# f90/Wave-U-Net

Measured on AMD Instinct MI355X. Metric: waveform samples/sec fwd+bwd, M1 12-level Wave-U-Net @1/2/4/8 GPU, higher is better.
Workload: dtype f32

## Files before the change

wave-u-net_amd/csrc/wun_dispatch.hip:

```cpp
#include "wun_plan_impl.h"

#include <algorithm>
#include <cstdio>
#include <cstdlib>
#include <cstring>
#include <functional>
#include <string>
#include <vector>

ConvArgs conv_base(const wun_plan* p) {
    ConvArgs a;
    memset(&a, 0, sizeof(a));
    a.B = p->B; a.ostride = 1; a.loader = LOADER_DIRECT;
    return a;
}
void set_src0(ConvArgs& a, const float* ws, const Buf& b, int off, int C) {
    a.src0 = ws + b.off; a.bs0 = b.bs; a.pitch0 = b.pitch; a.off0 = off; a.C0 = C;
}
void set_src1(ConvArgs& a, const float* ws, const Buf& b, int off, int C) {
    a.src1 = ws + b.off; a.bs1 = b.bs; a.pitch1 = b.pitch; a.off1 = off; a.C1 = C;
}
void set_dst0(ConvArgs& a, float* ws, const Buf& b, int off, const Buf* mask) {
    a.dst0 = ws + b.off; a.obs0 = b.bs; a.opitch0 = b.pitch; a.ooff0 = off;
    a.msk0 = mask ? ws + mask->off : nullptr;
// ... 155 lines not shown
                }
                vec[idx] = bc;
                if (p->sw.tune_log)
                    fprintf(stderr, "[tune conv-bf16 %s#%zu] C=%d N=%d T=%d K=%d ld=%d ph2=%d cands=%d base %.3f ms -> code=%d %.3f ms\n",
                            p->in_bwd ? "bwd" : "fwd", idx, a.C0 + a.C1, a.N, a.Tout, a.KW, a.loader, (a.flags & F_PHASE2) ? 1 : 0, n,
                            base, bc.variant, best);
            }
            if (p->tune_mode >= 1 && idx < vec.size() && vec[idx].variant >= kBf16VariantBase && conv_bf16_choice_ok(a, vec[idx].variant))
                a.force_variant = vec[idx].variant + 1;
            return launch_conv_bf16(a, s, p->sw);
        }
    }
    if (p->tune_mode == 1) {
        if (vec.size() <= idx) vec.resize(idx + 1, ConvChoice{-1, 0});
        std::vector<ConvChoice> cands_v(640);
        std::vector<float> tms_v(641);
        ConvChoice* cands = cands_v.data();
        float* tms = tms_v.data();
        const int n = conv_list_candidates(a, part ? cap : 0, cands, 640, p->sw);
        time_candidates(p, s, n + 1, [&](int i) {
            ConvArgs b = a;
            b.ups_y = nullptr; b.ubw_dz = nullptr;
            if (i < n) { b.force_variant = cands[i].variant + 1; b.force_ksplit = cands[i].ksplit; }
            return launch_conv(b, part, cap, s, p->sw);
        }, tms);
        const float base = tms[n];
        float best = base;
        ConvChoice bc{-1, 0};
        int bi = -1;
        for (int i = 0; i < n; ++i)
            if (bi < 0 ? tms[i] < 1e29f : tms[i] < tms[bi]) bi = i;
        if (bi >= 0 && tms[bi] < base * 0.98f) { best = tms[bi]; bc = cands[bi]; }
        vec[idx] = bc;
        char head[96];
        snprintf(head, sizeof(head), "%s %zu %d %d %.4f\n", p->in_bwd ? "cb" : "cf", idx, -1, 0, base);
        tune_alts(p, head, tms, (size_t)n, best, base, [&](FILE* f, size_t i) {
            fprintf(f, "%s %zu %d %d %.4f\n", p->in_bwd ? "cb" : "cf", idx, cands[i].variant, cands[i].ksplit, tms[i]);
        });
        if (p->sw.tune_log)
            fprintf(stderr, "[tune conv %s#%zu] C=%d N=%d T=%d K=%d ld=%d ph2=%d cands=%d base %.3f ms -> v=%d ks=%d %.3f ms\n",
                    p->in_bwd ? "bwd" : "fwd", idx, a.C0 + a.C1, a.N, a.Tout, a.KW, a.loader, (a.flags & F_PHASE2) ? 1 : 0, n,
                    base, bc.variant, bc.ksplit, best);
    }
    if (p->tune_mode >= 1 && idx < vec.size() && vec[idx].variant >= 0 &&
        conv_choice_ok(a, part ? cap : 0, vec[idx].variant, vec[idx].ksplit > 0 ? vec[idx].ksplit : 1, p->sw)) {
        a.force_variant = vec[idx].variant + 1; a.force_ksplit = vec[idx].ksplit;
    }
    return launch_conv(a, part, cap, s, p->sw);
}

static bool wgrad_common_geom(WgradArgs* parts, int nparts, int mtw, int nw) {
    int m0 = 0, n0 = 0;
    for (int i = 0; i < nparts; ++i) {
        parts[i].force_mtw = mtw; parts[i].force_nw = nw;
        int m, n;
        wgrad_resolved_geom(parts[i], m, n);
        if (i == 0) { m0 = m; n0 = n; }
        else if (m != m0 || n != n0) return false;
    }
    return true;
}

int run_wgrad(const wun_plan* p, WgradArgs* parts, int nparts, const ConvLayer& cl, float* ws,
                     float* grads, hipStream_t main, hipStream_t s, bool dep, bool accum) {
    if (dep) {
        int rcd = stream_dep(p, main, s);
        if (rcd) return rcd;
    }
    if (p->bf16) {
        if (!wgrad_bf16_supported(parts[0])) return fail(WUN_ERR_UNSUPPORTED, "bf16 mode: weight-gradient shape not served by the bf16 kernel");
        for (int i = 0; i < nparts; ++i) { parts[i].bf16 = 1; parts[i].sbf = 1; }
// ... 186 lines not shown
```

wave-u-net_amd/csrc/wun_internal.h:

```cpp
#pragma once
#include <hip/hip_runtime.h>
#include <stdint.h>
#include <string>

namespace wun {

enum { LOADER_DIRECT = 0, LOADER_DEINT = 1 };

enum WunEarlyWindow { EW_DEFAULT, EW_OFF, EW_DEEP, EW_ALL };
enum WunEventScope { EV_DEFAULT, EV_SYSTEM, EV_DEVICE };
enum WunSidePrio { PRIO_DEFAULT, PRIO_LOW, PRIO_HIGH, PRIO_NORMAL };
struct WunSwitches {
    bool no_dedup = false;
    WunEarlyWindow early_window = EW_DEFAULT;
    bool odd_fuse_set = false;
    int odd_fuse_min = 64;
    bool no_odd_align = false;
    bool no_fuse_ups = false;
    bool bf16_head_serial = false;
    bool single_stream = false;
    WunSidePrio side_prio = PRIO_DEFAULT;
    WunEventScope event_scope = EV_DEFAULT;
    bool no_win = false;
    bool no_narrow = false;
    bool no_narrow_down0 = false;
    bool no_narrow_stream = false;
    int narrow_splits = 0;
    bool no_dma = false;
    bool no_k3 = false;
    int win_tk = 64;
    int bf16_lds_cap = 80;
    int tune_rounds = 4;
    bool tune_log = false;
    std::string tune_alts;
    int tune_alts_max = 6;
    float tune_alts_tol = 1.15f;
    bool dump_layout = false;
    bool profile_detail = false;
    bool win_occ = false;
};
WunSwitches wun_switches_from_env();

enum { F_LRELU = 1, F_ACCUM = 2, F_VEC4 = 4, F_PHASE2 = 8 };

struct ConvArgs {
    const float* src0; const float* src1;
    long long bs0, bs1;
    int pitch0, pitch1;
    int off0, off1;
    int C0, C1;
    int Tin;
    int shift;
// ... 7 lines not shown
    int opitch0, opitch1;
    int ooff0, ooff1;
    const float* msk0; const float* msk1;
    int ostride;
    int Tout;
    float* dec; long long decbs; int decpitch;
    int dec_exp; int dec_lo; unsigned dec_len;
    float* dec1; long long dec1bs; int dec1pitch;
    int dec_off, dec1_off;
    int flags;
    int B;
    int loader;
    int Tlim;
    int kw_full;
    int force_variant;
    int force_ksplit;
    int cps;
    float* part;
    int wb_c8p, wb_npad;
    int acc_lo; unsigned acc_len;
    float* ups_y; long long ups_bs; int ups_pitch; int ups_tup; const float* ups_w;
    float* ubw_dz; const float* ubw_x; long long ubw_bs; int ubw_pitch; int ubw_n;
    int xbf, obf;
};
#define WUN_FIRST_RETIRED_VARIANT 42
#define WUN_NUM_RETIRED_VARIANTS 14
int conv_last_fused_ups();
static inline bool aligned16(const void* p) { return (reinterpret_cast<uintptr_t>(p) & 15) == 0; }
void conv_output_setup(ConvArgs& a);

struct WgradArgs {
    const float* src0; const float* src1;
    long long bs0, bs1;
    int pitch0, pitch1;
    int off0, off1;
    int C0, C1;
    int Tin;
    int shift;
    int KW;
    int loader;
    const float* dz; long long dzbs; int dzpitch; int N; int Tq;
    float* out;
    int direct;
    int split_base;
    int nsplit; int units_per_split; int nQT; int B;
    int ablate;
    int force_mtw, force_nw;
// ... 81 lines not shown
    int C, B, Tin;
    const float* dpre; long long dps, dpbs; int dppitch;
    const float* Wh; long long hoff[4]; int Sh, Ko, padl, Tfeat, Tout, moff_feat;
    const float* dlast; int moff_diff;
    float* dmix;
};

struct PackDesc {
    long long src_off;
    long long dst_off;
    int KW, C, N, C8p, Npad;
    int src_in_ws;
};

struct WtDesc {
    long long src_off;
    long long dst_off;
    int J, C, N, k_last, k_step;
    int mode;
};

size_t conv_lds_bytes(const ConvArgs& a, int variant, const WunSwitches& sw);
int  conv_pick_variant(const ConvArgs& a);
hipError_t launch_conv(const ConvArgs& a, float* part, long long part_cap, hipStream_t s, const WunSwitches& sw);
double conv_flops(const ConvArgs& a);
long long conv_natural_wgs_phase2(const ConvArgs& a);
int conv_list_candidates(const ConvArgs& a, long long part_cap, ConvChoice* out, int maxn, const WunSwitches& sw);
bool conv_choice_ok(const ConvArgs& a, long long part_cap, int variant, int ksplit, const WunSwitches& sw);
int conv_num_variants();
int wgrad_max_units(const WgradArgs& a, const WunSwitches& sw);

int  wgrad_pick_nsplit(const WgradArgs& a, const WunSwitches& sw);
hipError_t launch_wgrad(const WgradArgs& a, hipStream_t s, const WunSwitches& sw);
void wgrad_resolved_geom(const WgradArgs& a, int& mtw, int& nw);
long long wgrad_partial_floats(const WgradArgs& a, const WunSwitches& sw);
hipError_t launch_wgrad_reduce(const WgradArgs& a, const float* partial, int nsplit, float* out_w, float* out_b,
                               hipStream_t s, const WunSwitches& sw);
enum { EW_UPSAMPLE = 0, EW_UPSAMPLE_BWD, EW_INTERP_GRAD, EW_HEAD_FWD, EW_HEAD_DFEAT, EW_BTC_TO_NCW, EW_NUM_OPS };
enum { EW_PATH_NONE = 0, EW_PATH_SCALAR, EW_PATH_VEC4, EW_PATH_VEC8_BF16, EW_PATH_ONE_STAGE, EW_PATH_TWO_STAGE,
       EW_PATH_GENERIC, EW_PATH_FOUR_POSITION };
int elementwise_last_path(int op);
hipError_t launch_upsample(const UpsampleArgs& a, hipStream_t s);
hipError_t launch_upsample_bwd(const UpsampleBwdArgs& a, hipStream_t s);
hipError_t launch_interp_grad(const UpsampleBwdArgs& a, hipStream_t s, bool accum = false);
hipError_t launch_head_fwd_off(const HeadArgs& a, const long long* hoff, hipStream_t s);
int head_bwd_blocks(const HeadArgs& a);
hipError_t launch_head_bwd_off(const HeadArgs& a, const long long* hoff, hipStream_t s);
// ... 78 lines not shown
```

wave-u-net_amd/csrc/wun_kernels.hip:

```cpp
#include "wun_device.h"

#include <cstdio>
#include <cstdlib>
#include <map>
#include <mutex>
#include <string>
#include <algorithm>
#include <vector>

namespace wun {

__device__ __forceinline__ f32x4 mfma16(float a, float b, f32x4 c) {
    return __builtin_amdgcn_mfma_f32_16x16x4f32(a, b, c, 0, 0, 0);
}

__host__ __device__ static inline int fit_pitch(int width, int mod32) {
    return width + (((mod32 - (width % 32)) % 32) + 32) % 32;
}

struct ProfSlot { std::string name; std::string tag; double flops; double bytes; hipEvent_t e0, e1, c0, c1; };
static std::vector<ProfSlot> g_prof;
static bool g_prof_on = false;
static bool g_prof_detail = false;
static std::mutex g_prof_mu;
// ... 72 lines not shown
    }
    g_prof.clear();
    double overhead_ms = 0.0;
    if (!empty_ms.empty()) {
        std::sort(empty_ms.begin(), empty_ms.end());
        overhead_ms = empty_ms[empty_ms.size() / 2];
    }
    char obuf[96];
    snprintf(obuf, sizeof(obuf), "{\"bracket_overhead_ms\": %.6f, ", overhead_ms);
    std::string out = std::string(obuf) + "\"launches\": [" + detail + "], \"kernels\": [";
    bool first = true;
    for (auto& kv : agg) {
        char buf[512];
        snprintf(buf, sizeof(buf), "%s{\"name\": \"%s\", \"launches\": %ld, \"ms\": %.6f, \"flops\": %.6e, \"bytes\": %.6e}",
                 first ? "" : ", ", kv.first.c_str(), kv.second.n, kv.second.ms, kv.second.flops, kv.second.bytes);
        out += buf;
        first = false;
    }
    out += "]}";
    return out;
}

#define WUN_JMAX 15


__device__ __forceinline__ int fast_div(int n, int d, float inv) {
    int q = (int)(((float)n + 0.5f) * inv);
    const int r = n - q * d;
    q += (r >= d) ? 1 : 0;
    q -= (r < 0) ? 1 : 0;
    return q;
}

#define WUN_FOLD_XCAP(TT) (3 * (TT) + 32)

__device__ __forceinline__ void conv_copy1(const ConvArgs& a, int b, int n, int q, float v) {
    if (a.dec != nullptr) {
        float* row = a.dec + (long long)b * a.decbs + (long long)n * a.decpitch + a.dec_off;
        if (a.dec_exp) {
            const unsigned pos = (unsigned)(2 * q - a.dec_lo);
            if (pos < a.dec_len) row[pos] = v;
        } else if ((q & 1) == 0) {
            row[q >> 1] = v;
        }
    }
    if (a.dec1 != nullptr && (q & 1) != 0) a.dec1[(long long)b * a.dec1bs + (long long)n * a.dec1pitch + a.dec1_off + (q >> 1)] = v;
// ... 23 lines not shown
    extern __shared__ __attribute__((aligned(16))) float lds_all[];
    const int kg = KG > 1 ? __builtin_amdgcn_readfirstlane((int)(threadIdx.x >> 8)) : 0;
    constexpr int TT = WT * MT * 16;
    constexpr int NT = WN * NW * 16;
    constexpr int NT4 = NT / 4;
    constexpr int CH = CK / 2;
    constexpr int TPR = 256 / CK;
    constexpr int XIT_D = FOLD ? (WUN_FOLD_XCAP(TT) + TPR - 1) / TPR : (TT + WUN_JMAX - 1 + TPR - 1) / TPR;
    constexpr int TPC = 256 / CH;
    constexpr int XIT_I = FOLD ? (2 * WUN_FOLD_XCAP(TT) + TPC - 1) / TPC
                               : (2 * (TT + (WUN_JMAX + 1) / 2 - 1) + TPC - 1) / TPC;
    constexpr int XIT = XVEC ? 1 : (XIT_D > XIT_I ? XIT_D : XIT_I);
    constexpr int WIT = XVEC ? 1 : (WUN_JMAX * CK * NT4 + 255) / 256;
    constexpr int XDIT = XVEC ? (CK * ((TT + 48) / 4) + 255) / 256 : 1;
    constexpr int WDIT = XVEC ? (WUN_JMAX * CK * (NT4 + 4) + 255) / 256 : 1;
    static_assert(!(XVEC && FOLD), "DMA staging is not implemented for batch-folded tiles");

    const int XB = CK * XP, LB = CK * XP + J * CK * WP;
    float* lds = lds_all + (KG > 1 ? kg * 2 * LB : 0);
    float* Xs = lds;
    float* Ws = lds + XB;

    const int tid = KG > 1 ? (int)(threadIdx.x & 255) : (int)threadIdx.x;
    const int lane = tid & 63;
    const int li = lane & 15, lg = lane >> 4;
    const int wave = __builtin_amdgcn_readfirstlane(tid >> 6);
#define WUN_PRIO_HI() __builtin_amdgcn_s_setprio(2)
#define WUN_PRIO_LO() __builtin_amdgcn_s_setprio(0)
    WUN_PRIO_HI();
    int bid = xcd_contiguous_block((int)blockIdx.x, (int)gridDim.x);
    const int nt = bid % nNT; bid /= nNT;
    const int tt = bid % nTT; bid /= nTT;
    const float inv_tout = 1.0f / (float)a.Tout;
    const int b = FOLD ? fast_div(tt * TT, a.Tout, inv_tout) : bid % a.B;
    const int ksg = FOLD ? bid : bid / a.B;
    const int ksp = ksg * KG + kg;
    const int q0 = tt * TT, n0 = nt * NT;
    int fold_nb = 1;
    const int fold_seg = a.Tout + J - 1;
    if constexpr (FOLD) {
        int last = fast_div(q0 + TT - 1, a.Tout, inv_tout);
        if (last > a.B - 1) last = a.B - 1;
        fold_nb = last - b + 1;
    }
    const int wt0 = (wave % WT) * MT * 16;
    const int wn0 = (wave / WT) * NW * 16;
// ... 19 lines not shown

    float xreg[XIT];
    f32x4 wreg[WIT];
    unsigned xmask = 0, wmask = 0;

    int xt[XIT];
    unsigned xmask_s = 0, wmask_s = 0;
    const int xrow = deint ? tid / TPC : tid / TPR;
    const int dl0 = XVEC ? (((a.off0 - a.shift) % 4) + 4) % 4 : 0;
    const int dl1 = (XVEC && a.C1 > 0) ? (((a.off1 - a.shift) % 4) + 4) % 4 : dl0;
    int xdo[XDIT], wdo[WDIT];
    int nvr = 1, e00 = 0, e01 = 0;
    bool xedge = false;
    const float* vb0 = a.src0 + (long long)b * a.bs0;
    const float* vb1 = (a.src1 != nullptr) ? a.src1 + (long long)b * a.bs1 : vb0;
    const int XG = XP >> 2, WG4 = WP >> 2;
    if constexpr (XVEC) {
        const int tbase = q0 - a.shift;
        nvr = (UW + (dl0 > dl1 ? dl0 : dl1) + 3) >> 2;
        e00 = a.off0 + tbase - dl0;
        e01 = a.off1 + tbase - dl1;
        const int tf0 = tbase - dl0, tf1 = tbase - dl1;
        xedge = tf0 < 0 || tf0 + 4 * nvr > a.Tin || (a.C1 > 0 && (tf1 < 0 || tf1 + 4 * nvr > a.Tin));
        const float inv_xg = 1.0f / (float)XG;
#pragma unroll
        for (int i = 0; i < XDIT; ++i) {
            const int f = tid + i * 256;
            const int row = fast_div(f, XG, inv_xg), g = f - row * XG;
            xdo[i] = (row < CK && g < nvr) ? (row << 20) | (4 * g) : -1;
        }
        const float inv_wg = 1.0f / (float)WG4;
#pragma unroll
        for (int i = 0; i < WDIT; ++i) {
            const int f = tid + i * 256;
            const int row = fast_div(f, WG4, inv_wg), c4 = f - row * WG4;
            const int j = row / CK, r = row - j * CK;
            const bool ok = j < J && c4 < NT4;
            int wo;
            if (!phase2) {
                int col = n0 + c4 * 4;
                col = col > a.N - 4 ? a.N - 4 : col;
                wo = (j * Ctot + r) * a.N + col;
            } else {
                const int x = c4 * 4, ph = x / (NT / 2), cl = x % (NT / 2);
                int col = n0h + cl;
                col = col > a.N - 4 ? a.N - 4 : col;
                wo = (j * Ctot + r) * (2 * a.N) + ph * a.N + col;
            }
            wdo[i] = ok ? wo : -1;
        }
    }
    if constexpr (!XVEC) {
        const int lr = deint ? tid % TPC : tid % TPR;
        const int stride_i = deint ? TPC : TPR;
        const int lim = deint ? 2 * UW : UW;
        const int tbase = (deint ? 2 * q0 : q0) - a.shift;
        const int seglen = deint ? 2 * fold_seg : fold_seg;
        const float inv_seglen = 1.0f / (float)seglen;
#pragma unroll
        for (int i = 0; i < XIT; ++i) {
            const int u = lr + i * stride_i;
            int t = tbase + u, bl = 0;
            if constexpr (FOLD) { bl = fast_div(u, seglen, inv_seglen); t = u - bl * seglen - a.shift; }
            const bool ok = u < lim && t >= 0 && t < a.Tin;
            int tc = t < 0 ? 0 : t;
            if (tc > a.Tin - 1) tc = a.Tin - 1;
            if constexpr (FOLD) {
                if (bl > fold_nb - 1) bl = fold_nb - 1;
                tc |= bl << 20;
            }
            xt[i] = tc;
            xmask_s |= (ok ? 1u : 0u) << i;
// ... 678 lines not shown
    if (!aligned16(a.src0) || (a.bs0 & 3) != 0 || (a.pitch0 & 3) != 0 || a.pitch0 < 4) return false;
    if (a.src1 != nullptr && (!aligned16(a.src1) || (a.bs1 & 3) != 0 || (a.pitch1 & 3) != 0 || a.pitch1 < 4)) return false;
    if (a.off0 < 0 || a.off1 < 0 || !aligned16(a.W)) return false;
    if ((long long)cv.CK * a.pitch0 >= (1ll << 31) || (long long)cv.CK * a.pitch1 >= (1ll << 31)) return false;
    return true;
}

static void conv_geom(const ConvArgs& a, int variant, const WunSwitches& sw, int& TT, int& NT, int& J, int& XP, int& WP) {
    const ConvVariant& v = kConvVariants[variant];
    TT = v.WT * v.MT * 16;
    NT = v.WN * v.NW * 16;
    J = conv_J(a);
    XP = fit_pitch(v.fold ? WUN_FOLD_XCAP(TT) : TT + J - 1, 16);
    if (conv_xvec_ok(a, variant, sw)) XP = conv_dma_pitch(TT + J - 1 + 3);
    WP = fit_pitch(NT, 16);
}

static inline long long conv_mtiles(const ConvArgs& a, int variant, int TT, int& bfac) {
    if (kConvVariants[variant].fold) { bfac = 1; return ((long long)a.B * a.Tout + TT - 1) / TT; }
    bfac = a.B;
    return (a.Tout + TT - 1) / TT;
}

size_t conv_lds_bytes(const ConvArgs& a, int variant, const WunSwitches& sw) {
    if (is_k3(variant)) {
        const int bv = conv_tile_variant(variant);
        const size_t stage = WUN_KG * conv_lds_bytes(a, bv, sw);
        const size_t red = (size_t)(WUN_KG - 1) * kConvVariants[bv].MT * kConvVariants[bv].NW * 256 * 16;
        return stage > red ? stage : red;
    }
    if (variant >= WUN_FIRST_RETIRED_VARIANT) return (size_t)1 << 30;
    int TT, NT, J, XP, WP;
    conv_geom(a, variant, sw, TT, NT, J, XP, WP);
    const int CK = kConvVariants[variant].CK;
    return 2 * sizeof(float) * ((size_t)CK * XP + (size_t)J * CK * WP);
}

double conv_flops(const ConvArgs& a) {
    if (a.flags & F_PHASE2)
        return 2.0 * a.kw_full * (double)(a.C0 + a.C1) * a.N * (double)a.Tin * a.B;
    return 2.0 * a.KW * (double)(a.C0 + a.C1) * a.N * (double)a.Tout * a.B;
}

void conv_splitk(const ConvArgs& a, int variant, const WunSwitches& sw, long long part_cap_floats, int& ksplit, int& cps) {
    int TT, NT, J, XP, WP;
    conv_geom(a, variant, sw, TT, NT, J, XP, WP);
// ... 43 lines not shown
        const int CKC = a.loader == LOADER_DEINT ? CK / 2 : CK;
        const int nchunks = (a.C0 + a.C1 + CKC - 1) / CKC;
        int want = a.force_ksplit > nchunks ? nchunks : a.force_ksplit;
        if (part == nullptr) want = 1;
        const long long per = (long long)a.B * a.N * ((a.Tout + 3) & ~3);
        if (want > 1 && (long long)want * per > part_cap) return hipErrorInvalidValue;
        cps = (nchunks + want - 1) / want;
        ksplit = (nchunks + cps - 1) / cps;
    }
    if (KG > 1) {
        const int CKC = a.loader == LOADER_DEINT ? CK / 2 : CK;
        const int nchunks = (a.C0 + a.C1) / CKC;
        const int want = (a.force_ksplit > 0 && part != nullptr) ? a.force_ksplit : 1;
        if ((a.C0 + a.C1) % CKC != 0 || nchunks % (KG * want) != 0) return hipErrorInvalidValue;
        const long long per = (long long)a.B * a.N * ((a.Tout + 3) & ~3);
        if (want > 1 && (long long)want * per > part_cap) return hipErrorInvalidValue;
        ksplit = want;
        cps = nchunks / (KG * want);
    }
    a.cps = cps;
    a.part = ksplit > 1 ? part : nullptr;
    const long long grid = (long long)nTT * nNT * bfac * ksplit;
    if (grid <= 0) return hipSuccess;
    char nm[64];
    snprintf(nm, sizeof(nm), "conv_mfma_kernel<%d, %d, %d, %d, %d, %s%s%s%s>", MT, NW, WT, WN, CK, VECW ? "true" : "false",
             FOLD ? ", fold" : "", XVEC ? ", dma" : "", KG > 1 ? ", k3" : "");
    {
        char tag[160];
        snprintf(tag, sizeof(tag), "C=%d N=%d T=%d K=%d ld=%d B=%d ks=%d ph2=%d acc=%d os=%d grid=%lld", a.C0 + a.C1, a.N,
                 a.Tout, a.KW, a.loader, a.B, ksplit, (a.flags & F_PHASE2) ? 1 : 0, (a.flags & F_ACCUM) ? 1 : 0,
                 a.ostride, grid);
        ProfScope ps(nm, conv_flops(a), s, tag);
        hipLaunchKernelGGL(kern, dim3((unsigned)grid), dim3(256 * KG), lds_launch, s, a, nTT, nNT, J, XP, WP);
    }
    hipError_t e = hipGetLastError();
    if (e != hipSuccess || ksplit == 1) return e;
    const long long total = (long long)a.B * a.N * (((a.Tout + 3) & ~3) >> 2);
    long long blocks = (total + 255) / 256;
    if (blocks > 4096) blocks = 4096;
    {
        const double elems = (double)a.B * a.N * a.Tout;
        double by = 4.0 * elems * (ksplit + 1 + (a.msk0 != nullptr ? 1 : 0) + ((a.flags & F_ACCUM) ? 1 : 0));
        if (a.ups_y != nullptr) by += 4.0 * (double)a.B * a.N * a.ups_tup;
        ProfScope ps("conv_splitk_epilogue_kernel", 0.0, s, "", by);
        hipLaunchKernelGGL(conv_splitk_epilogue_kernel, dim3((unsigned)blocks), dim3(256), 0, s, a, ksplit);
    }
// ... 48 lines not shown

int conv_list_candidates(const ConvArgs& a, long long part_cap, ConvChoice* out, int maxn, const WunSwitches& sw) {
    int n = 0;
    const int nvar = conv_num_variants();
    static const int ks_menu[] = {1, 2, 3, 4, 6, 8, 12, 16, 24, 32, 48};
    for (int v = 0; v < nvar && n < maxn; ++v)
        for (unsigned i = 0; i < sizeof(ks_menu) / sizeof(ks_menu[0]) && n < maxn; ++i) {
            if (!conv_choice_ok(a, part_cap, v, ks_menu[i], sw)) {
                if (is_k3(v) && ks_menu[i] < 8) continue;
                break;
            }
            out[n].variant = v; out[n].ksplit = ks_menu[i]; ++n;
        }
    return n;
}

static_assert(sizeof(kConvVariants) / sizeof(kConvVariants[0]) == WUN_FIRST_RETIRED_VARIANT, "the retired index range follows the tile table");
static int first_k3_variant() { return WUN_FIRST_RETIRED_VARIANT + WUN_NUM_RETIRED_VARIANTS; }
int conv_num_variants() { return first_k3_variant() + kNumK3; }


int conv_last_fused_ups() { return t_last_fused_ups; }

hipError_t launch_conv(const ConvArgs& a_in, float* part, long long part_cap, hipStream_t s, const WunSwitches& sw) {
    ConvArgs a = a_in;
    t_last_fused_ups = 0;
    if (a.ups_y != nullptr && (a.dst1 != nullptr || a.msk0 != nullptr || a.ostride != 1 || a.ooff0 != 0 ||
                               (a.flags & (F_ACCUM | F_PHASE2)) != 0 || a.N0 != a.N || !aligned16(a.ups_y)))
        return hipErrorInvalidValue;
    if (a.ubw_dz != nullptr && (a.dst1 == nullptr || a.msk1 != nullptr || a.ostride != 1 || a.bias != nullptr ||
                                (a.flags & (F_ACCUM | F_PHASE2 | F_LRELU)) != 0 || a.N0 >= a.N || a.ubw_x == nullptr))
        return hipErrorInvalidValue;
    conv_output_setup(a);
    if (conv_J(a) > WUN_JMAX) return hipErrorInvalidValue;
    if (a.KW <= 0) {
        const long long total = (long long)a.B * a.N * (((a.Tout + 3) & ~3) >> 2);
        if (total <= 0) return hipSuccess;
        long long blocks = (total + 255) / 256;
        if (blocks > 4096) blocks = 4096;
        hipLaunchKernelGGL(conv_splitk_epilogue_kernel, dim3((unsigned)blocks), dim3(256), 0, s, a, 0);
        return hipGetLastError();
    }
    const bool vecw = (a.N & 3) == 0 && aligned16(a.W);
    if ((a.flags & F_PHASE2) && !(a.ostride == 1 && a.dst1 == nullptr && vecw)) return hipErrorInvalidValue;
    int v = (a.flags & F_PHASE2) ? conv_pick_variant_phase2(a) : conv_pick_variant(a);
    if (a.force_variant > 0 && vecw) {
        v = a.force_variant - 1;
        if (!conv_choice_ok(a, part != nullptr ? part_cap : 0, v, a.force_ksplit > 0 ? a.force_ksplit : 1, sw)) return hipErrorInvalidValue;
    }
// ... 567 lines not shown
```

wave-u-net_amd/csrc/wun_op.hip:

```cpp
#include "wun_plan_impl.h"

#include <algorithm>
#include <cstdio>
#include <cstdlib>
#include <cstring>

namespace wun {
hipError_t launch_make_wt_one(const float* src, float* dst, WtDesc d, hipStream_t s);
}

static const long long kOpScratchFloats = 8ll << 20;
static int g_op_variant = -1, g_op_ksplit = 0;
static int g_op_wg_mtw = 0, g_op_wg_nw = 0, g_op_wg_nsplit = 0;
static int g_op_wg_bf16 = 0;
static int g_op_wg_narrow = 0;
static int g_op_wg_win = 0;
static float* g_op_copy0 = nullptr; static float* g_op_copy1 = nullptr;
static int g_op_copy_t0 = 0, g_op_copy_t1 = 0, g_op_copy_exp = 0, g_op_copy_lo = 0, g_op_copy_len = 0, g_op_acc_lo = 0, g_op_acc_len = 0;
static float* g_op_ups_y = nullptr; static const float* g_op_ups_w = nullptr;
static int g_op_ups_pitch = 0, g_op_ups_tup = 0;
static thread_local int t_op_epilogue_path = WUN_PATH_NONE;
static float* op_scratch() {
    static float* buf = nullptr;
    if (!buf && hipMalloc((void**)&buf, kOpScratchFloats * sizeof(float)) != hipSuccess) {
// ... 4 lines not shown
}

static void* op_bf16_tmp(int slot, size_t bytes) {
    static void* buf[2] = {nullptr, nullptr};
    static size_t cap[2] = {0, 0};
    if (bytes > cap[slot]) {
        (void)hipDeviceSynchronize();
        if (buf[slot]) (void)hipFree(buf[slot]);
        buf[slot] = nullptr; cap[slot] = 0;
        const size_t want = bytes + (bytes >> 2) + 4096;
        if (hipMalloc(&buf[slot], want) != hipSuccess) { (void)hipGetLastError(); return nullptr; }
        cap[slot] = want;
    }
    return buf[slot];
}
static inline int pad8(int t) { return (t + 7) / 8 * 8; }
static const float* op_to_bf16(int slot, const float* src, long long rows, int T, long long spitch, hipStream_t s) {
    void* dst = op_bf16_tmp(slot, (size_t)rows * pad8(T) * 2 + 64);
    if (!dst) return nullptr;
    if (launch_cast_rows_bf16(src, dst, rows, T, spitch, pad8(T), s) != hipSuccess) return nullptr;
    return reinterpret_cast<const float*>(dst);
}

static hipError_t op_launch_conv(ConvArgs a, hipStream_t s) {
    if (g_op_variant >= 0) { a.force_variant = g_op_variant + 1; a.force_ksplit = (a.flags & F_PHASE2) ? 0 : g_op_ksplit; }
    return launch_conv(a, op_scratch(), kOpScratchFloats, s, wun_switches_from_env());
}

static void op_src(ConvArgs& a, const float* x, int C, int T) {
    const int pitch = T;
    a.src0 = x; a.bs0 = (long long)C * pitch; a.pitch0 = pitch; a.off0 = 0; a.C0 = C;
}

extern "C" int wun_op_conv1d(const float* x, const float* w, const float* bias, float* y, int batch, int cin,
                             int cout, int k, int t_in, int t_out, int stride, int pad_left, int lrelu,
                             void* stream) {
    if (!x || !w || !y) return fail(WUN_ERR_INVALID, "null argument");
    if (stride != 1 && stride != 2) return fail(WUN_ERR_UNSUPPORTED, "stride must be 1 or 2");
    ConvArgs a;
    memset(&a, 0, sizeof(a));
    a.B = batch; a.ostride = 1;
    op_src(a, x, cin, t_in);
    a.loader = stride == 2 ? LOADER_DEINT : LOADER_DIRECT;
    a.Tin = t_in; a.shift = pad_left; a.W = w; a.bias = bias; a.KW = k; a.N = a.N0 = cout; a.Tout = t_out;
    a.flags = lrelu ? F_LRELU : 0;
    a.dst0 = y; a.obs0 = (long long)cout * t_out; a.opitch0 = t_out;
    HIP_TRY(op_launch_conv(a, (hipStream_t)stream));
    return WUN_OK;
}
// ... 167 lines not shown
extern "C" int wun_op_set_wgrad_bf16(int on) { g_op_wg_bf16 = on ? 1 : 0; return WUN_OK; }
extern "C" int wun_op_set_wgrad_win(int on) { g_op_wg_win = on ? 1 : 0; return WUN_OK; }
extern "C" int wun_op_set_wgrad_narrow(int on) { g_op_wg_narrow = on ? 1 : 0; return WUN_OK; }

extern "C" int wun_op_force_wgrad_variant(int mtw, int nw, int nsplit) {
    g_op_wg_mtw = mtw; g_op_wg_nw = nw; g_op_wg_nsplit = nsplit;
    return WUN_OK;
}

extern "C" int wun_op_conv1d_ex(const float* x0, int c0, const float* x1, int c1, const float* w, const float* bias,
                                float* y, const float* mask, int batch, int cout, int k, int t_in, int t_out,
                                int t_y, int stride, int pad_left, int lrelu, int accumulate, int ostride, int ooff,
                                void* stream) {
    if (!x0 || !w || !y) return fail(WUN_ERR_INVALID, "null argument");
    if (stride != 1 && stride != 2) return fail(WUN_ERR_UNSUPPORTED, "stride must be 1 or 2");
    if (c0 < 1 || c1 < 0 || (c1 > 0 && !x1)) return fail(WUN_ERR_INVALID, "bad source channels");
    if (ostride < 1 || ooff < 0 || (long long)(t_out - 1) * ostride + ooff >= t_y) return fail(WUN_ERR_INVALID, "output does not fit t_y");
    ConvArgs a;
    memset(&a, 0, sizeof(a));
    a.B = batch; a.ostride = ostride;
    a.src0 = x0; a.bs0 = (long long)c0 * t_in; a.pitch0 = t_in; a.C0 = c0;
    if (c1 > 0) { a.src1 = x1; a.bs1 = (long long)c1 * t_in; a.pitch1 = t_in; a.C1 = c1; }
    a.loader = stride == 2 ? LOADER_DEINT : LOADER_DIRECT;
    a.Tin = t_in; a.shift = pad_left; a.W = w; a.bias = bias; a.KW = k; a.N = a.N0 = cout; a.Tout = t_out;
    a.flags = (lrelu ? F_LRELU : 0) | (accumulate ? F_ACCUM : 0);
    a.dst0 = y; a.obs0 = (long long)cout * t_y; a.opitch0 = t_y; a.ooff0 = ooff; a.msk0 = mask;
    if (g_op_copy0 != nullptr) {
        a.dec = g_op_copy0; a.decpitch = g_op_copy_t0; a.decbs = (long long)cout * g_op_copy_t0;
        a.dec_exp = g_op_copy_exp; a.dec_lo = g_op_copy_lo; a.dec_len = (unsigned)g_op_copy_len;
    }
    if (g_op_copy1 != nullptr) { a.dec1 = g_op_copy1; a.dec1pitch = g_op_copy_t1; a.dec1bs = (long long)cout * g_op_copy_t1; }
    if (accumulate && g_op_acc_len > 0) { a.acc_lo = g_op_acc_lo; a.acc_len = (unsigned)g_op_acc_len; }
    if (g_op_ups_y != nullptr) {
        if (g_op_ups_tup != 2 * t_out - 1 && g_op_ups_tup != 2 * t_out) return fail(WUN_ERR_INVALID, "ups_tup must be 2 t_out - 1 or 2 t_out");
        if (stride != 1 || ostride != 1 || ooff != 0 || accumulate || mask) return fail(WUN_ERR_INVALID, "fused upsampling: plain forward launches only");
        if ((reinterpret_cast<uintptr_t>(g_op_ups_y) & 15) != 0) return fail(WUN_ERR_INVALID, "fused upsampling: ups_y must be 16-byte aligned");
        a.ups_y = g_op_ups_y; a.ups_pitch = g_op_ups_pitch; a.ups_bs = (long long)cout * g_op_ups_pitch;
        a.ups_tup = g_op_ups_tup; a.ups_w = g_op_ups_w;
    }
    HIP_TRY(op_launch_conv(a, (hipStream_t)stream));
    if (a.ups_y != nullptr) {
        t_op_epilogue_path = conv_last_fused_ups() ? WUN_PATH_FUSED : WUN_PATH_NOT_FUSED;
        if (!conv_last_fused_ups()) {
            UpsampleArgs u;
            memset(&u, 0, sizeof(u));
            u.x = y; u.xpitch = t_y; u.xbs = (long long)cout * t_y; u.n = t_out;
            u.y = a.ups_y; u.ypitch = a.ups_pitch; u.ybs = a.ups_bs; u.tup = a.ups_tup; u.w = a.ups_w;
// ... 281 lines not shown
```

wave-u-net_amd/csrc/wun_plan.hip:

```cpp
#include "wun_plan_impl.h"

#include <cmath>
#include <cstdio>
#include <cstdlib>
#include <cstring>
#include <algorithm>
#include <string>
#include <vector>

thread_local std::string g_err;
bool g_profiling = false;

int fail(int code, const std::string& msg) {
    g_err = msg;
    return code;
}

WunSwitches wun::wun_switches_from_env() {
    WunSwitches w;
    auto set = [](const char* name) { return getenv(name) != nullptr; };
    auto num = [](const char* name, int dflt) { const char* e = getenv(name); return e ? atoi(e) : dflt; };
    w.no_dedup = set("WUN_NO_DEDUP");
    if (const char* e = getenv("WUN_EARLY_WINDOW")) w.early_window = e[0] == '0' ? EW_OFF : e[0] == 'a' ? EW_ALL : EW_DEEP;
    w.odd_fuse_set = set("WUN_ODD_FUSE_MIN");
    w.odd_fuse_min = num("WUN_ODD_FUSE_MIN", 64);
    w.no_odd_align = set("WUN_NO_ODD_ALIGN");
    w.no_fuse_ups = set("WUN_NO_FUSE_UPS");
    w.bf16_head_serial = set("WUN_BF16_HEAD_SERIAL");
    w.single_stream = set("WUN_SINGLE_STREAM");
    if (const char* e = getenv("WUN_SIDE_PRIO")) w.side_prio = e[0] == 'l' ? PRIO_LOW : e[0] == 'h' ? PRIO_HIGH : PRIO_NORMAL;
    if (const char* e = getenv("WUN_EVENT_SCOPE")) w.event_scope = e[0] == 's' ? EV_SYSTEM : e[0] == 'd' ? EV_DEVICE : EV_DEFAULT;
    w.no_win = set("WUN_NO_WIN");
    w.no_narrow = set("WUN_NO_NARROW");
    w.no_narrow_down0 = set("WUN_NO_NARROW_DOWN0");
    w.no_narrow_stream = num("WUN_NO_NARROW_STREAM", 0) != 0;
    if (set("WUN_NARROW_SPLITS")) w.narrow_splits = std::max(1, num("WUN_NARROW_SPLITS", 0));
    w.no_dma = set("WUN_NO_DMA");
    w.no_k3 = num("WUN_NO_K3", 0) != 0;
    { const int v = num("WUN_WIN_TK", 64); if (v == 16 || v == 32 || v == 64 || v == 128) w.win_tk = v; }
    w.bf16_lds_cap = num("WUN_BF16_LDS_CAP", 80);
    w.tune_rounds = std::max(1, num("WUN_TUNE_ROUNDS", 4));
    w.tune_log = set("WUN_TUNE_LOG");
    if (const char* e = getenv("WUN_TUNE_ALTS")) w.tune_alts = e;
    { const int v = num("WUN_TUNE_ALTS_MAX", 6); w.tune_alts_max = v > 0 ? v : 6; }
    if (const char* e = getenv("WUN_TUNE_ALTS_TOL")) { const float v = (float)atof(e); w.tune_alts_tol = v > 1.f ? v : 1.15f; }
    w.dump_layout = set("WUN_DUMP_LAYOUT");
    w.profile_detail = set("WUN_PROFILE_DETAIL");
    w.win_occ = set("WUN_WIN_OCC");
    return w;
}

static int check_config(const wun_config* c) {
    if (!c) return fail(WUN_ERR_INVALID, "config is null");
    if (c->num_layers < 1 || c->num_layers > 24) return fail(WUN_ERR_INVALID, "num_layers out of range");
    if (c->num_initial_filters < 1) return fail(WUN_ERR_INVALID, "num_initial_filters < 1");
    if (c->filter_size < 1 || c->merge_filter_size < 1 || c->output_filter_size < 1 || c->input_filter_size < 1)
        return fail(WUN_ERR_INVALID, "filter sizes must be >= 1");
    if (c->filter_size > 15 || c->merge_filter_size > 15)
        return fail(WUN_ERR_UNSUPPORTED, "filter_size / merge_filter_size > 15 not supported by the gfx950 kernels");
    if (c->upsampling != 0 && c->upsampling != 1) return fail(WUN_ERR_UNSUPPORTED, "upsampling must be linear|learned");
    if (c->output_type != 0 && c->output_type != 1) return fail(WUN_ERR_UNSUPPORTED, "output_type must be direct|difference");
// ... 481 lines not shown
```

wave-u-net_amd/csrc/wun_plan_impl.h:

```cpp
#pragma once
#include "../../include/wun.h"
#include "wun_internal.h"

#include <cstring>
#include <map>
#include <string>
#include <vector>

using namespace wun;

struct Buf { long long off = -1; int C = 0; int T = 0; int pitch = 0; long long bs = 0; int eb = 4; };
struct ConvLayer { long long woff = 0, boff = 0; int KW = 0, Cin = 0, Cout = 0;
                   long long wt_full = -1, wt_ph[2] = {-1, -1}, wt_ph2 = -1; int Jp[2] = {0, 0}; int J0 = 0;
                   long long wt_ph2s = -1; int J0s = 0; };
struct DownShape { int cin, cout, t_in, t_conv, t_dec, tc, cs, t_ev0, n_even, t_odd0, n_odd; };
struct UpShape { int c_skip, c_cur, cout, t_cur, t_up, t_conv, crop_start; };

struct wun_plan {
    wun_config cfg;
    WunSwitches sw;
    WunEarlyWindow early_window = EW_DEEP;
    bool fuse_ups = false;
    int B = 0, Tin = 0, Tout = 0;
    int L = 0, C = 0, S = 0, Sh = 0;
// ... 27 lines not shown
    mutable std::vector<ConvChoice> conv_fwd, conv_bwd;
    mutable std::vector<WgradChoice> wg_bwd;
    mutable size_t ci = 0, wi = 0;
    mutable bool in_bwd = false;
    mutable hipEvent_t tev0 = nullptr, tev1 = nullptr;
    mutable hipStream_t side = nullptr, side2 = nullptr;
    mutable std::vector<hipEvent_t> events;
    mutable size_t ev_next = 0;
    mutable hipEvent_t wt_ev = nullptr;
    mutable bool wt_ready = false;
    mutable std::vector<hipEvent_t> skip_ev;
    mutable std::vector<hipEvent_t> win_ev;
    struct BfImg { long long off; int c8p, npad; };
    bool bf16 = false;
    std::map<std::pair<int, long long>, BfImg> bf_img;
    std::vector<PackDesc> pack;
    int npack_fwd = 0;
    long long pack_max = 0;
    PackDesc* dev_pack = nullptr;
    std::vector<NormChunk> norm_chunks;
    std::vector<int> norm_first;
    NormChunk* dev_norm_chunks = nullptr;
    int* dev_norm_first = nullptr;
    mutable const float* cur_params = nullptr;
    mutable const float* cur_ws = nullptr;
};

struct DownPart { int off, Tin, shift, stride, loader; const Buf* dz; int Tq; };
inline int down_parts(const wun_plan* p, int i, DownPart out[2]) {
    const DownShape& d = p->dsh[i];
    const int Kd = p->cfg.filter_size;
    if (p->same) {
        out[0] = DownPart{0, d.t_in, (Kd - 1) / 2, 1, LOADER_DIRECT, &p->dz_skip[i], d.t_conv};
        return 1;
    }
    out[0] = DownPart{0, d.t_in, 0, 2, LOADER_DEINT, &p->dz_dec[i], d.t_dec};
    if (p->dedup) {
        out[1] = DownPart{d.t_odd0, d.t_in - d.t_odd0, 0, 2, LOADER_DEINT, &p->dz_odd[i], d.n_odd};
        return d.n_odd > 0 ? 2 : 1;
    }
    out[1] = DownPart{d.cs, d.tc + Kd - 1, 0, 1, LOADER_DIRECT, &p->dz_skip[i], d.tc};
    return 2;
}

extern thread_local std::string g_err;
extern bool g_profiling;
// ... 45 lines not shown
```

Measured before the change: 33.08 million.

## Precompute per-thread DMA staging offsets into cached device lookup tables

```diff
diff --git a/wave-u-net_amd/csrc/wun_dispatch.hip b/wave-u-net_amd/csrc/wun_dispatch.hip
--- a/wave-u-net_amd/csrc/wun_dispatch.hip
+++ b/wave-u-net_amd/csrc/wun_dispatch.hip
@@ -201,7 +201,7 @@
             ConvArgs b = a;
             b.ups_y = nullptr; b.ubw_dz = nullptr;
             if (i < n) { b.force_variant = cands[i].variant + 1; b.force_ksplit = cands[i].ksplit; }
-            return launch_conv(b, part, cap, s, p->sw);
+            return launch_conv(b, part, cap, s, p->sw, &p->stage);
         }, tms);
         const float base = tms[n];
         float best = base;
@@ -225,7 +225,7 @@
         conv_choice_ok(a, part ? cap : 0, vec[idx].variant, vec[idx].ksplit > 0 ? vec[idx].ksplit : 1, p->sw)) {
         a.force_variant = vec[idx].variant + 1; a.force_ksplit = vec[idx].ksplit;
     }
-    return launch_conv(a, part, cap, s, p->sw);
+    return launch_conv(a, part, cap, s, p->sw, &p->stage);
 }
 
 static bool wgrad_common_geom(WgradArgs* parts, int nparts, int mtw, int nw) {
diff --git a/wave-u-net_amd/csrc/wun_internal.h b/wave-u-net_amd/csrc/wun_internal.h
--- a/wave-u-net_amd/csrc/wun_internal.h
+++ b/wave-u-net_amd/csrc/wun_internal.h
@@ -1,6 +1,7 @@
 #pragma once
 #include <hip/hip_runtime.h>
 #include <stdint.h>
+#include <string.h>
 #include <string>
 
 namespace wun {
@@ -28,6 +29,7 @@
     int narrow_splits = 0;
     bool no_dma = false;
     bool no_k3 = false;
+    bool no_stage_table = false;
     int win_tk = 64;
     int bf16_lds_cap = 80;
     int tune_rounds = 4;
@@ -81,7 +83,37 @@
     float* ups_y; long long ups_bs; int ups_pitch; int ups_tup; const float* ups_w;
     float* ubw_dz; const float* ubw_x; long long ubw_bs; int ubw_pitch; int ubw_n;
     int xbf, obf;
-};
+    const int* stage;
+};
+
+struct StageGeom {
+    int TT, NT, CK;
+    int J, XP, WP;
+    int Ctot, N;
+    int phase2;
+    int nvr;
+};
+inline bool operator<(const StageGeom& x, const StageGeom& y) { return memcmp(&x, &y, sizeof(StageGeom)) < 0; }
+static inline int stage_xdit(const StageGeom& g) { return (g.CK * ((g.TT + 48) / 4) + 255) / 256; }
+static inline int stage_wdit(const StageGeom& g) { return (15 * g.CK * (g.NT / 4 + 4) + 255) / 256; }
+static inline int stage_quads(const StageGeom& g) { return (stage_xdit(g) + stage_wdit(g) + 3) / 4; }
+long long stage_table_build(const StageGeom& g, int32_t* out, long long cap);
+class StageCache {
+public:
+    StageCache();
+    ~StageCache();
+    StageCache(const StageCache&) = delete;
+    StageCache& operator=(const StageCache&) = delete;
+    const int* get(const StageGeom& g);
+    long long device_bytes() const;
+private:
+    struct Impl;
+    Impl* d;
+};
+struct WunSwitches;
+bool conv_stage_geom(const ConvArgs& a, int variant, const WunSwitches& sw, StageGeom& g);
+long long stage_table_launches();
+void stage_table_count_launch();
 #define WUN_FIRST_RETIRED_VARIANT 42
 #define WUN_NUM_RETIRED_VARIANTS 14
 int conv_last_fused_ups();
@@ -209,7 +241,8 @@
 
 size_t conv_lds_bytes(const ConvArgs& a, int variant, const WunSwitches& sw);
 int  conv_pick_variant(const ConvArgs& a);
-hipError_t launch_conv(const ConvArgs& a, float* part, long long part_cap, hipStream_t s, const WunSwitches& sw);
+hipError_t launch_conv(const ConvArgs& a, float* part, long long part_cap, hipStream_t s, const WunSwitches& sw,
+                       StageCache* stage = nullptr);
 double conv_flops(const ConvArgs& a);
 long long conv_natural_wgs_phase2(const ConvArgs& a);
 int conv_list_candidates(const ConvArgs& a, long long part_cap, ConvChoice* out, int maxn, const WunSwitches& sw);
diff --git a/wave-u-net_amd/csrc/wun_kernels.hip b/wave-u-net_amd/csrc/wun_kernels.hip
--- a/wave-u-net_amd/csrc/wun_kernels.hip
+++ b/wave-u-net_amd/csrc/wun_kernels.hip
@@ -118,6 +118,9 @@
 }
 
 #define WUN_JMAX 15
+#ifndef WUN_STAGE_ALWAYS
+#define WUN_STAGE_ALWAYS 0
+#endif
 
 
 __device__ __forceinline__ int fast_div(int n, int d, float inv) {
@@ -187,6 +190,19 @@
     float* Ws = lds + XB;
 
     const int tid = KG > 1 ? (int)(threadIdx.x & 255) : (int)threadIdx.x;
+    constexpr int STQ = XVEC ? (XDIT + WDIT + 3) / 4 : 1;
+    int stg[4 * STQ];
+    const bool staged = XVEC && (WUN_STAGE_ALWAYS || a.stage != nullptr);
+    if constexpr (XVEC) {
+        if (staged) {
+            const int4* tab = reinterpret_cast<const int4*>(a.stage) + tid;
+#pragma unroll
+            for (int q = 0; q < STQ; ++q) {
+                const int4 v = tab[q * 256];
+                stg[4 * q] = v.x; stg[4 * q + 1] = v.y; stg[4 * q + 2] = v.z; stg[4 * q + 3] = v.w;
+            }
+        }
+    }
     const int lane = tid & 63;
     const int li = lane & 15, lg = lane >> 4;
     const int wave = __builtin_amdgcn_readfirstlane(tid >> 6);
@@ -252,32 +268,45 @@
         e01 = a.off1 + tbase - dl1;
         const int tf0 = tbase - dl0, tf1 = tbase - dl1;
         xedge = tf0 < 0 || tf0 + 4 * nvr > a.Tin || (a.C1 > 0 && (tf1 < 0 || tf1 + 4 * nvr > a.Tin));
-        const float inv_xg = 1.0f / (float)XG;
-#pragma unroll
-        for (int i = 0; i < XDIT; ++i) {
-            const int f = tid + i * 256;
-            const int row = fast_div(f, XG, inv_xg), g = f - row * XG;
-            xdo[i] = (row < CK && g < nvr) ? (row << 20) | (4 * g) : -1;
-        }
-        const float inv_wg = 1.0f / (float)WG4;
-#pragma unroll
-        for (int i = 0; i < WDIT; ++i) {
-            const int f = tid + i * 256;
-            const int row = fast_div(f, WG4, inv_wg), c4 = f - row * WG4;
-            const int j = row / CK, r = row - j * CK;
-            const bool ok = j < J && c4 < NT4;
-            int wo;
-            if (!phase2) {
-                int col = n0 + c4 * 4;
+        if (staged) {
+            const int ncol0 = phase2 ? n0h : n0;
+#pragma unroll
+            for (int i = 0; i < XDIT; ++i) xdo[i] = stg[i];
+#pragma unroll
+            for (int i = 0; i < WDIT; ++i) {
+                const int pk = stg[XDIT + i];
+                int col = ncol0 + (pk & 127);
                 col = col > a.N - 4 ? a.N - 4 : col;
-                wo = (j * Ctot + r) * a.N + col;
-            } else {
-                const int x = c4 * 4, ph = x / (NT / 2), cl = x % (NT / 2);
-                int col = n0h + cl;
-                col = col > a.N - 4 ? a.N - 4 : col;
-                wo = (j * Ctot + r) * (2 * a.N) + ph * a.N + col;
-            }
-            wdo[i] = ok ? wo : -1;
+                wdo[i] = pk >= 0 ? (pk >> 7) + col : -1;
+            }
+        } else {
+            const float inv_xg = 1.0f / (float)XG;
+#pragma unroll
+            for (int i = 0; i < XDIT; ++i) {
+                const int f = tid + i * 256;
+                const int row = fast_div(f, XG, inv_xg), g = f - row * XG;
+                xdo[i] = (row < CK && g < nvr) ? (row << 20) | (4 * g) : -1;
+            }
+            const float inv_wg = 1.0f / (float)WG4;
+#pragma unroll
+            for (int i = 0; i < WDIT; ++i) {
+                const int f = tid + i * 256;
+                const int row = fast_div(f, WG4, inv_wg), c4 = f - row * WG4;
+                const int j = row / CK, r = row - j * CK;
+                const bool ok = j < J && c4 < NT4;
+                int wo;
+                if (!phase2) {
+                    int col = n0 + c4 * 4;
+                    col = col > a.N - 4 ? a.N - 4 : col;
+                    wo = (j * Ctot + r) * a.N + col;
+                } else {
+                    const int x = c4 * 4, ph = x / (NT / 2), cl = x % (NT / 2);
+                    int col = n0h + cl;
+                    col = col > a.N - 4 ? a.N - 4 : col;
+                    wo = (j * Ctot + r) * (2 * a.N) + ph * a.N + col;
+                }
+                wdo[i] = ok ? wo : -1;
+            }
         }
     }
     if constexpr (!XVEC) {
@@ -1002,6 +1031,21 @@
     return (a.Tout + TT - 1) / TT;
 }
 
+static thread_local StageCache* t_stage_cache = nullptr;
+bool conv_stage_geom(const ConvArgs& a, int variant, const WunSwitches& sw, StageGeom& g) {
+    variant = conv_tile_variant(variant);
+    if (variant < 0 || variant >= WUN_FIRST_RETIRED_VARIANT || !conv_xvec_ok(a, variant, sw)) return false;
+    memset(&g, 0, sizeof(g));
+    conv_geom(a, variant, sw, g.TT, g.NT, g.J, g.XP, g.WP);
+    g.CK = kConvVariants[variant].CK;
+    g.Ctot = a.C0 + a.C1; g.N = a.N;
+    g.phase2 = (a.flags & F_PHASE2) ? 1 : 0;
+    const int dl0 = (((a.off0 - a.shift) % 4) + 4) % 4;
+    const int dl1 = a.C1 > 0 ? (((a.off1 - a.shift) % 4) + 4) % 4 : dl0;
+    g.nvr = (g.TT + g.J - 1 + (dl0 > dl1 ? dl0 : dl1) + 3) >> 2;
+    return true;
+}
+
 size_t conv_lds_bytes(const ConvArgs& a, int variant, const WunSwitches& sw) {
     if (is_k3(variant)) {
         const int bv = conv_tile_variant(variant);
@@ -1091,6 +1135,12 @@
     a.part = ksplit > 1 ? part : nullptr;
     const long long grid = (long long)nTT * nNT * bfac * ksplit;
     if (grid <= 0) return hipSuccess;
+    a.stage = nullptr;
+    if (XVEC && t_stage_cache != nullptr && !sw.no_stage_table) {
+        StageGeom sg;
+        if (conv_stage_geom(a, variant, sw, sg)) a.stage = t_stage_cache->get(sg);
+        if (a.stage != nullptr) stage_table_count_launch();
+    }
     char nm[64];
     snprintf(nm, sizeof(nm), "conv_mfma_kernel<%d, %d, %d, %d, %d, %s%s%s%s>", MT, NW, WT, WN, CK, VECW ? "true" : "false",
              FOLD ? ", fold" : "", XVEC ? ", dma" : "", KG > 1 ? ", k3" : "");
@@ -1185,9 +1235,11 @@
 
 int conv_last_fused_ups() { return t_last_fused_ups; }
 
-hipError_t launch_conv(const ConvArgs& a_in, float* part, long long part_cap, hipStream_t s, const WunSwitches& sw) {
+hipError_t launch_conv(const ConvArgs& a_in, float* part, long long part_cap, hipStream_t s, const WunSwitches& sw,
+                       StageCache* stage) {
     ConvArgs a = a_in;
     t_last_fused_ups = 0;
+    t_stage_cache = stage;
     if (a.ups_y != nullptr && (a.dst1 != nullptr || a.msk0 != nullptr || a.ostride != 1 || a.ooff0 != 0 ||
                                (a.flags & (F_ACCUM | F_PHASE2)) != 0 || a.N0 != a.N || !aligned16(a.ups_y)))
         return hipErrorInvalidValue;
diff --git a/wave-u-net_amd/csrc/wun_op.hip b/wave-u-net_amd/csrc/wun_op.hip
--- a/wave-u-net_amd/csrc/wun_op.hip
+++ b/wave-u-net_amd/csrc/wun_op.hip
@@ -50,9 +50,35 @@
     return reinterpret_cast<const float*>(dst);
 }
 
+static StageCache* op_stage_cache() {
+    static StageCache* c = new StageCache;
+    return c;
+}
+static int g_op_crop0 = 0, g_op_crop1 = 0;
+
 static hipError_t op_launch_conv(ConvArgs a, hipStream_t s) {
     if (g_op_variant >= 0) { a.force_variant = g_op_variant + 1; a.force_ksplit = (a.flags & F_PHASE2) ? 0 : g_op_ksplit; }
-    return launch_conv(a, op_scratch(), kOpScratchFloats, s, wun_switches_from_env());
+    return launch_conv(a, op_scratch(), kOpScratchFloats, s, wun_switches_from_env(), op_stage_cache());
+}
+
+extern "C" int wun_stage_test_set_crop(int off0, int off1) {
+    if (off0 < 0 || off1 < 0) return fail(WUN_ERR_INVALID, "negative crop offset");
+    g_op_crop0 = off0; g_op_crop1 = off1;
+    return WUN_OK;
+}
+extern "C" int wun_stage_test_geom(int variant, int k, int c0, int c1, int cout, int off0, int off1, int pad_left, int phase2,
+                                   int pitch, int32_t* geom) {
+    if (!geom) return 0;
+    ConvArgs a;
+    memset(&a, 0, sizeof(a));
+    a.loader = LOADER_DIRECT; a.KW = k; a.C0 = c0; a.C1 = c1; a.N = a.N0 = cout; a.off0 = off0; a.off1 = off1;
+    a.shift = pad_left; a.flags = phase2 ? F_PHASE2 : 0;
+    a.pitch0 = a.pitch1 = pitch; a.bs0 = (long long)c0 * pitch; a.bs1 = (long long)c1 * pitch;
+    StageGeom g;
+    WunSwitches sw;
+    if (variant < 0 || variant >= conv_num_variants() || !conv_stage_geom(a, variant, sw, g)) return 0;
+    memcpy(geom, &g, sizeof(g));
+    return 1;
 }
 
 static void op_src(ConvArgs& a, const float* x, int C, int T) {
@@ -266,7 +292,12 @@
     a.src0 = x0; a.bs0 = (long long)c0 * t_in; a.pitch0 = t_in; a.C0 = c0;
     if (c1 > 0) { a.src1 = x1; a.bs1 = (long long)c1 * t_in; a.pitch1 = t_in; a.C1 = c1; }
     a.loader = stride == 2 ? LOADER_DEINT : LOADER_DIRECT;
-    a.Tin = t_in; a.shift = pad_left; a.W = w; a.bias = bias; a.KW = k; a.N = a.N0 = cout; a.Tout = t_out;
+    a.Tin = t_in; a.shift = pad_left;
+    if (g_op_crop0 > 0 || g_op_crop1 > 0) {
+        if (std::max(g_op_crop0, g_op_crop1) >= t_in) return fail(WUN_ERR_INVALID, "crop offset beyond the row");
+        a.off0 = g_op_crop0; a.off1 = c1 > 0 ? g_op_crop1 : 0; a.Tin = t_in - std::max(g_op_crop0, g_op_crop1);
+    }
+    a.W = w; a.bias = bias; a.KW = k; a.N = a.N0 = cout; a.Tout = t_out;
     a.flags = (lrelu ? F_LRELU : 0) | (accumulate ? F_ACCUM : 0);
     a.dst0 = y; a.obs0 = (long long)cout * t_y; a.opitch0 = t_y; a.ooff0 = ooff; a.msk0 = mask;
     if (g_op_copy0 != nullptr) {
diff --git a/wave-u-net_amd/csrc/wun_plan.hip b/wave-u-net_amd/csrc/wun_plan.hip
--- a/wave-u-net_amd/csrc/wun_plan.hip
+++ b/wave-u-net_amd/csrc/wun_plan.hip
@@ -37,6 +37,7 @@
     if (set("WUN_NARROW_SPLITS")) w.narrow_splits = std::max(1, num("WUN_NARROW_SPLITS", 0));
     w.no_dma = set("WUN_NO_DMA");
     w.no_k3 = num("WUN_NO_K3", 0) != 0;
+    w.no_stage_table = set("WUN_NO_STAGE_TABLE");
     { const int v = num("WUN_WIN_TK", 64); if (v == 16 || v == 32 || v == 64 || v == 128) w.win_tk = v; }
     w.bf16_lds_cap = num("WUN_BF16_LDS_CAP", 80);
     w.tune_rounds = std::max(1, num("WUN_TUNE_ROUNDS", 4));
diff --git a/wave-u-net_amd/csrc/wun_plan_impl.h b/wave-u-net_amd/csrc/wun_plan_impl.h
--- a/wave-u-net_amd/csrc/wun_plan_impl.h
+++ b/wave-u-net_amd/csrc/wun_plan_impl.h
@@ -73,6 +73,7 @@
     std::vector<int> norm_first;
     NormChunk* dev_norm_chunks = nullptr;
     int* dev_norm_first = nullptr;
+    mutable StageCache stage;
     mutable const float* cur_params = nullptr;
     mutable const float* cur_ws = nullptr;
 };
diff --git a/wave-u-net_amd/csrc/wun_stage.hip b/wave-u-net_amd/csrc/wun_stage.hip
--- /dev/null
+++ b/wave-u-net_amd/csrc/wun_stage.hip
@@ -0,0 +1,106 @@
+#include "wun_internal.h"
+
+#include <atomic>
+#include <map>
+#include <mutex>
+#include <vector>
+
+namespace wun {
+
+long long stage_table_build(const StageGeom& g, int32_t* out, long long cap) {
+    const int XDIT = stage_xdit(g), WDIT = stage_wdit(g), Q = stage_quads(g);
+    const long long need = (long long)Q * 1024;
+    if (out == nullptr || cap < need) return 0;
+    if (g.TT < 16 || g.NT < 16 || g.CK < 1 || g.J < 1 || g.XP < 4 || g.WP < 4 || g.Ctot < 1 || g.N < 4 || g.nvr < 1) return 0;
+    if (g.CK >= (1 << 10) || g.XP >= (1 << 20) || g.NT > 128) return 0;
+    const long long wrows = (long long)g.J * g.Ctot * g.N * (g.phase2 ? 2 : 1);
+    if (wrows >= (1ll << 24)) return 0;
+    const int XG = g.XP >> 2, WG4 = g.WP >> 2, NT4 = g.NT / 4;
+    for (int tid = 0; tid < 256; ++tid) {
+        for (int e = 0; e < 4 * Q; ++e) {
+            int32_t v = -1;
+            if (e < XDIT) {
+                const int f = tid + e * 256;
+                const int row = f / XG, gr = f - row * XG;
+                if (row < g.CK && gr < g.nvr) v = (row << 20) | (4 * gr);
+            } else if (e - XDIT < WDIT) {
+                const int f = tid + (e - XDIT) * 256;
+                const int row = f / WG4, c4 = f - row * WG4;
+                const int j = row / g.CK, r = row - j * g.CK;
+                if (j < g.J && c4 < NT4) {
+                    if (!g.phase2) {
+                        v = (((j * g.Ctot + r) * g.N) << 7) | (c4 * 4);
+                    } else {
+                        const int x = c4 * 4, ph = x / (g.NT / 2), cl = x % (g.NT / 2);
+                        v = (((j * g.Ctot + r) * (2 * g.N) + ph * g.N) << 7) | cl;
+                    }
+                }
+            }
+            out[((long long)(e >> 2) * 256 + tid) * 4 + (e & 3)] = v;
+        }
+    }
+    return need;
+}
+
+static std::atomic<long long> g_stage_launches{0};
+long long stage_table_launches() { return g_stage_launches.load(); }
+void stage_table_count_launch() { g_stage_launches.fetch_add(1); }
+
+struct StageCache::Impl {
+    static constexpr size_t kSlabBytes = 1 << 20;
+    std::mutex mu;
+    std::map<StageGeom, const int*> tab;
+    std::vector<char*> slabs;
+    size_t used = kSlabBytes;
+};
+
+StageCache::StageCache() : d(new Impl) {}
+StageCache::~StageCache() {
+    for (char* s : d->slabs) (void)hipFree(s);
+    delete d;
+}
+long long StageCache::device_bytes() const {
+    std::lock_guard<std::mutex> lk(d->mu);
+    return (long long)d->slabs.size() * (long long)Impl::kSlabBytes;
+}
+
+const int* StageCache::get(const StageGeom& g) {
+    std::lock_guard<std::mutex> lk(d->mu);
+    auto it = d->tab.find(g);
+    if (it != d->tab.end()) return it->second;
+    const int* dev = nullptr;
+    std::vector<int32_t> host((size_t)stage_quads(g) * 1024);
+    const long long n = stage_table_build(g, host.data(), (long long)host.size());
+    const size_t bytes = (size_t)n * sizeof(int32_t);
+    if (n > 0 && bytes <= Impl::kSlabBytes) {
+        if (d->used + bytes > Impl::kSlabBytes) {
+            char* slab = nullptr;
+            if (hipMalloc((void**)&slab, Impl::kSlabBytes) == hipSuccess) { d->slabs.push_back(slab); d->used = 0; }
+            else (void)hipGetLastError();
+        }
+        if (d->used + bytes <= Impl::kSlabBytes) {
+            char* dst = d->slabs.back() + d->used;
+            if (hipMemcpy(dst, host.data(), bytes, hipMemcpyHostToDevice) == hipSuccess) {
+                dev = reinterpret_cast<const int*>(dst);
+                d->used += (bytes + 255) & ~(size_t)255;
+            } else {
+                (void)hipGetLastError();
+            }
+        }
+    }
+    d->tab[g] = dev;
+    return dev;
+}
+
+}
+
+extern "C" long long wun_stage_table_build(const int32_t* geom, int32_t* out, long long cap, int32_t* dims) {
+    if (!geom) return 0;
+    wun::StageGeom g;
+    memcpy(&g, geom, sizeof(g));
+    if (g.TT < 16 || g.NT < 16 || g.CK < 1 || g.TT > (1 << 16) || g.NT > (1 << 16) || g.CK > (1 << 10)) return 0;
+    if (dims) { dims[0] = wun::stage_xdit(g); dims[1] = wun::stage_wdit(g); dims[2] = wun::stage_quads(g); }
+    if (!out) return (long long)wun::stage_quads(g) * 1024;
+    return wun::stage_table_build(g, out, cap);
+}
+extern "C" long long wun_stage_table_launches(void) { return wun::stage_table_launches(); }
```

After: 32.95 million. Within noise of the previous version (-0.4%).
